# andewx/dieselfluid

Measured on AMD Instinct MI355X. Metric: M particle-steps/sec, 16M-particle WCSPH dam-break; % HBM roofline, higher is better.
Workload: dtype f32; 1 GPU; WCSPH dam-break, 16003008 particles (n3=252), h=2dx, uniform-grid neighbours, density + pressure/viscosity force + integrate + walls, math=fast; particles=16003008, parallelism=single GPU

## Files before the change

### dieselfluid_amd/csrc/kernels_skin.hpp

```cpp
#pragma once

#include "kernels_tiled.hpp"

namespace dsl {

constexpr int kLEntries = 8;
constexpr int kLMaxChunks = 12;
constexpr int kLMaxEntries = kLMaxChunks * kLEntries - 1;
constexpr int kLBlock = 512;
constexpr unsigned int kLGlobal = 0xffffu;
constexpr float kSkinTauSteps = 16.0f;
constexpr int kLQuads = 14;
static_assert(kTRows * kLQuads <= kLBlock, "one quad per lane");

__global__ void k_skin_decide(SkinState* st) {
  const float d = __builtin_sqrtf(__uint_as_float(st->disp2_bits)) * (1.0f + 1.0e-6f);
  const bool rb = st->force != 0 || !(d <= st->budget);
  st->rebuild = rb ? 1 : 0;
  if (st->unlisted * 64 > st->n_live) st->give_up = 1;
  if (rb) {
    st->ids_sel ^= 1;
    st->n_rebuilds += 1;
    st->unlisted = 0;
    st->fields_own = st->fields_padded = 0u;
// ... 216 lines not shown
          tile_run(m, rr, tt.lx, j, je);
          const int g0 = m.row_gs[rr] - m.row_lds[rr];
          const float xi = p.x[g], yi = p.y[g], zi = p.z[g];
          for (int r0 = j; r0 < je; r0 += 32) {
            unsigned int w = 0u;
            const int top = r0 + 31;
            for (int r = r0; r < min(r0 + 32, je); ++r) {
              const float dx = xi - p.x[g0 + r], dy = yi - p.y[g0 + r], dz = zi - p.z[g0 + r];
              const float tq = __builtin_fmaf(-dist2<true>(dx, dy, dz), c.inv_hh, 1.0f);
              if (tq > wide_thr && r != tt.own) w |= 1u << (top - r);
            }
            enqueue(w, top);
          }
        }
      }
      const int n_own = 1 + total;
      const bool fits = masks && !too_many && n_own <= kLMaxChunks * kLEntries;
      if (masks && !fits) st->list_overflow = 1;
      int fields = fits ? n_own : 0;
      const int own_fields = fields;
      int wmax = 0;
#pragma unroll
      for (int bit = 6; bit >= 0; --bit) {
        const int cand = wmax | (1 << bit);
        if (__builtin_amdgcn_ballot_w64(fields >= cand) != 0ull) wmax = cand;
      }
      if constexpr (!SHARED) fields = fits ? wmax : 0;
      atomicAdd(&tile_fields[0], (unsigned int)own_fields);
      atomicAdd(&tile_fields[1], (unsigned int)fields);
      const int nch = (fields + kLEntries - 1) / kLEntries;
      const int nch_wave = (wmax + kLEntries - 1) / kLEntries;
      unsigned int b0 = 0u, b1 = 0u, b2 = 0u, b3 = 0u;
      unsigned int k0 = 0u, k1 = 0u, k2 = 0u, k3 = 0u;
      int qi = 0;
      unsigned int w = 0u, top = 0u;
      unsigned int wn = (fits && nq > 0) ? qword[0][tid] : 0u, tn = (fits && nq > 0) ? qtop[0][tid] : 0u;
      const int nq_live = fits ? nq : 0;
      for (int it = 0; it < nch_wave * kLEntries; ++it) {
        unsigned int entry = pad;
        if (it == 0) {
          entry = 0u;
        } else {
          if (w == 0u && qi < nq_live) {
            w = wn;
            top = tn;
            qi += 1;
            if (qi < nq_live) {
              wn = qword[qi][tid];
              tn = qtop[qi][tid];
            }
          }
          if (w != 0u) {
            const int b = __builtin_ctz(w);
            w &= w - 1u;
            entry = (top - (unsigned int)b) << 4;
          }
        }
        b0 = __builtin_amdgcn_alignbit(b1, b0, 16);
        b1 = __builtin_amdgcn_alignbit(b2, b1, 16);
        b2 = __builtin_amdgcn_alignbit(b3, b2, 16);
        b3 = (b3 >> 16) | (entry << 16);
        if ((it & (kLEntries - 1)) == kLEntries - 1) {
          const int ch = it >> 3;
          if (ch == 0) {
            k0 = b0, k1 = b1, k2 = b2, k3 = b3;
          } else if (ch < nch) {
            lists[(size_t)ch * lstride + g] = make_uint4(b0, b1, b2, b3);
          }
        }
      }
      if (fits) lists[g] = make_uint4((k0 & 0xffff0000u) | (unsigned int)fields, k1, k2, k3);
      else lists[g] = make_uint4(kLGlobal, 0u, 0u, 0u);
    });
    if (have) tile_meta_store(metas[cur ^ 1], table_word);
    sync_lds();
    if (tid == 0) {
      atomicAdd(&st->fields_own, tile_fields[0]);
      atomicAdd(&st->fields_padded, tile_fields[1]);
      tile_fields[0] = tile_fields[1] = 0u;
    }
  }
}

template <int NF, class Load4, class Store>
__device__ __forceinline__ void stage_tile(const TileMeta& m, Load4&& load4, Store&& store) {
  const int t = threadIdx.x, r = t / kLQuads, k = t - r * kLQuads;
  if (r >= kTRows) return;
  const int len = m.row_len[r], gs = m.row_gs[r], ls = m.row_lds[r];
  for (int q = k; 4 * q < len; q += kLQuads) {
    float4 v[NF];
    load4(gs + 4 * q, v);
#pragma unroll
    for (int i = 0; i < 4; ++i) {
      if (4 * q + i < len) {
        float rec[NF];
#pragma unroll
        for (int a = 0; a < NF; ++a) rec[a] = f4_at(v[a], i);
        store(ls + 4 * q + i, rec, true);
      }
    }
  }
  const int npad = m.row_lds[r + 1] - ls - len;
  if (k < npad) {
    float rec[NF];
#pragma unroll
    for (int a = 0; a < NF; ++a) rec[a] = 0.0f;
    store(ls + len + k, rec, false);
  }
}

__device__ __forceinline__ const float4& lds_at(const float4* base, unsigned int byte_offset) {
  return *reinterpret_cast<const float4*>(reinterpret_cast<const char*>(base) + byte_offset);
}

struct Chunk {
  unsigned int x, y, z, w;
};
__device__ __forceinline__ Chunk load_chunk(const uint4* __restrict__ lists, size_t index) {
  const uint4 v = lists[index];
  return Chunk{v.x, v.y, v.z, v.w};
}
__device__ __forceinline__ Chunk pad_chunk(unsigned int pad) {
  const unsigned int w = pad | (pad << 16);
  return Chunk{w, w, w, w};
}
__device__ __forceinline__ unsigned int take_count(Chunk& e, unsigned int pad) {
  const unsigned int cnt = e.x & 0xffffu;
  e.x = (e.x & 0xffff0000u) | pad;
  return cnt;
}
__device__ __forceinline__ int chunks_of(unsigned int cnt) { return cnt == kLGlobal ? 0 : (int)((cnt + kLEntries) >> 3); }

template <class Body>
__device__ __forceinline__ void walk_shared(const uint4* __restrict__ lists, int lstride, int g, unsigned int pad, int sub,
                                            int k, unsigned int fields, Body&& body) {
  const int nch = fields == kLGlobal ? 0 : (int)((fields + kLEntries - 1) >> 3);
  for (int ch = sub; __builtin_amdgcn_ballot_w64(ch < nch) != 0ull; ch += k) {
    Chunk e = pad_chunk(pad);
    if (ch < nch) e = load_chunk(lists, (size_t)ch * lstride + g);
    if (ch == 0) e.x = (e.x & 0xffff0000u) | pad;
    body(e);
  }
}
__device__ __forceinline__ unsigned int shared_fields(const uint4* __restrict__ lists, int g, int sub) {
  unsigned int f = 0u;
  if (sub == 0) f = lists[g].x & 0xffffu;
  return (unsigned int)__shfl((int)f, (int)((threadIdx.x & (kWave - 1)) - sub), kWave);
}

__global__ __launch_bounds__(kLBlock, 4) void k_density_list(DevConsts c, TileGrid tg, const int* __restrict__ desc_of,
                                                             const int* __restrict__ n_tiles, const int* __restrict__ desc,
                                                             const int* __restrict__ cell_start, const SkinState* st,
                                                             CSoa3 pX, CSoa3 pZ, const uint4* __restrict__ lists,
                                                             int lstride, float* __restrict__ rho,
                                                             float* __restrict__ pterm) {
  __shared__ TileMeta metas[2];
  __shared__ float4 A[kTCap];
  const int tid = threadIdx.x;
  const CSoa3 p = st->rebuild ? pZ : pX;
  TileFeed feed(desc_of, *n_tiles);
  int di = 0;
  bool have = feed.pop(di);
  if (have) tile_meta_store(metas[0], tile_meta_request(desc, di));
  for (int cur = 0; have; cur ^= 1) {
    const TileMeta& m = metas[cur];
    sync_lds();
    have = feed.pop(di);
    int table_word = 0;
    if (have) table_word = tile_meta_request(desc, di);
    const int ntarg = m.tprefix[kTB * kTB];
    const bool staged = m.overflow == 0;
    const unsigned int pad = pad_entry(m);
    Chunk q0 = pad_chunk(pad), q1 = q0;
    const bool first_full = ntarg > kLBlock / 2;
    TileTarget tt0{0, 0, 0, 0};
    const int tperm = (tid & ~(kWave - 1)) + b128_group_slot(tid & (kWave - 1));
    if (first_full && tperm < ntarg) {
      tt0 = tile_target(m, tperm);
      q0 = load_chunk(lists, tt0.g);
      q1 = load_chunk(lists, (size_t)lstride + tt0.g);
    }
    if (staged) stage_tile<3>(m, LoadPos4{p}, StoreTileRecord(A, m, c.inv_hh));
    if (have) tile_meta_store(metas[cur ^ 1], table_word);
    sync_lds();
    for_each_target<true, kLBlock>(ntarg, tid, tperm, [&](auto shared_c, int t, int sub, int k) {
      constexpr bool SHARED = decltype(shared_c)::value;
      TileTarget tt;
      unsigned int fields;
      if constexpr (SHARED) {
        tt = tile_target(m, t);
        fields = shared_fields(lists, tt.g, sub);
      } else {
        if (t == tperm) tt = tt0;
        else {
          tt = tile_target(m, t);
          q0 = load_chunk(lists, tt.g);
          q1 = load_chunk(lists, (size_t)lstride + tt.g);
        }
        fields = take_count(q0, pad);
      }
      const int g = tt.g;
      float acc = 0.0f;
      if (staged && fields != kLGlobal) {
        const float4 me = A[tt.own];
        const float two_hh = 2.0f * c.inv_hh;
        const float sx = two_hh * me.x, sy = two_hh * me.y, sz = two_hh * me.z, a0 = 1.0f + me.w;
        float acc0 = 0.0f, acc1 = 0.0f;
        float4 cq[4];
        auto fetch4 = [&](unsigned int w0, unsigned int w1) {
          cq[0] = lds_at(A, w0 & 0xffffu);
          cq[1] = lds_at(A, w0 >> 16);
          cq[2] = lds_at(A, w1 & 0xffffu);
          cq[3] = lds_at(A, w1 >> 16);
        };
        auto sum4 = [&](const float4 (&r)[4]) {
#pragma unroll
          for (int u = 0; u < 4; ++u) {
            const float q = fma_clamp01(r[u].z, sz, __builtin_fmaf(r[u].y, sy, __builtin_fmaf(r[u].x, sx, r[u].w + a0)));
            if (u & 1) acc1 = __builtin_fmaf(q, q, acc1);
            else acc0 = __builtin_fmaf(q, q, acc0);
          }
        };
        if constexpr (SHARED) {
          walk_shared(lists, lstride, g, pad, sub, k, fields, [&](const Chunk& e) {
            fetch4(e.x, e.y);
            float4 c1[4] = {cq[0], cq[1], cq[2], cq[3]};
            fetch4(e.z, e.w);
            sum4(c1);
            sum4(cq);
          });
        } else {
          const int nf = __builtin_amdgcn_readfirstlane((int)fields), nch = (nf + kLEntries - 1) >> 3;
          const uint4* lp = lists + (size_t)2 * lstride + g;
          Chunk e = q0, e1 = q1;
          fetch4(e.x, e.y);
          for (int ch = 0;;) {
            float4 c1[4] = {cq[0], cq[1], cq[2], cq[3]};
            fetch4(e.z, e.w);
            sum4(c1);
            if (8 * ch + 4 >= nf) break;
            const Chunk en = e1;
            if (ch + 2 < nch) e1 = load_chunk(lp, 0);
            lp += lstride;
            float4 c2[4] = {cq[0], cq[1], cq[2], cq[3]};
            fetch4(en.x, en.y);
            sum4(c2);
            e = en;
            ch += 1;
            if (8 * ch >= nf) break;
          }
        }
        acc = acc0 + acc1;
      } else if (sub == 0) {
        const float xi = p.x[g], yi = p.y[g], zi = p.z[g];
        float a = 0.0f;
        for_each_grid_candidate(c, cell_start, xi, yi, zi, [&](int j) {
          if (j == g) return;
          const float dx = xi - p.x[j], dy = yi - p.y[j], dz = zi - p.z[j];
          const float r2 = dist2<true>(dx, dy, dz);
          if (r2 < c.hh) {
            const float q = __builtin_fmaf(-r2, c.inv_hh, 1.0f);
            a = __builtin_fmaf(q, q, a);
          }
        });
        acc = a;
      }
      if constexpr (SHARED) {
        for (int o = 1; o < k; o <<= 1) acc += __shfl_xor(acc, o, kWave);
        if (sub != 0) return;
      }
      acc *= c.mass * c.A;
      rho[g] = acc;
      const float pr = tait_eos<true>(c, acc, c.eos_d0_grad);
      pterm[g] = acc > 0.0f ? dsl_div<true>(pr, acc * acc) : 0.0f;
    });
  }
}

template <bool WANT_G, bool WANT_V, bool QUEUE>
__global__ __launch_bounds__(kLBlock, 4) void k_force_list(DevConsts c, TileGrid tg, const int* __restrict__ desc_of,
                                                           const int* __restrict__ n_tiles, const int* __restrict__ desc,
                                                           const int* __restrict__ cell_start, SkinState* st, CSoa3 pX,
                                                           CSoa3 vX, CSoa3 pZ, CSoa3 vZ, CSoa3 pR, const float* __restrict__ rho,
                                                           const float* __restrict__ pterm,
                                                           const uint4* __restrict__ lists, int lstride, Soa3 pout,
                                                           Soa3 vout, DevStats* stats, int* __restrict__ walk_ctr) {
  __shared__ TileMeta metas[2];
  __shared__ float4 A[kTCap];
  __shared__ float4 B[kTCap];
  __shared__ int feed_slot[2];
  const int tid = threadIdx.x;
  const bool rb = st->rebuild != 0;
  const CSoa3 pin = rb ? pZ : pX, vin = rb ? vZ : vX;
  unsigned int vbits = 0u, fbits = 0u, dbits = 0u;
  typename TileSource<QUEUE>::type feed = TileSource<QUEUE>::make(desc_of, *n_tiles, walk_ctr, feed_slot);
  int di = 0;
  bool have = feed.pop(di);
  if (have) tile_meta_store(metas[0], tile_meta_request(desc, di));
  for (int cur = 0; have; cur ^= 1) {
    const TileMeta& m = metas[cur];
    sync_lds();
    have = feed.pop(di);
    int table_word = 0;
    if (have) table_word = tile_meta_request(desc, di);
    const int ntarg = m.tprefix[kTB * kTB];
    const bool staged = m.overflow == 0;
    const unsigned int pad = pad_entry(m);
    Chunk q0 = pad_chunk(pad), q1 = q0;
    const bool first_full = ntarg > kLBlock / 2;
    TileTarget tt0{0, 0, 0, 0};
    const int tperm = (tid & ~(kWave - 1)) + b128_group_slot(tid & (kWave - 1));
    if (first_full && tperm < ntarg) {
      tt0 = tile_target(m, tperm);
      q0 = load_chunk(lists, tt0.g);
      q1 = load_chunk(lists, (size_t)lstride + tt0.g);
    }
    if (staged)
      stage_tile<8>(
          m,
          [&](int gg, float4* o) {
            o[0] = load4u(pin.x + gg);
            o[1] = load4u(pin.y + gg);
            o[2] = load4u(pin.z + gg);
            o[3] = WANT_G ? load4u(pterm + gg) : make_float4(0.f, 0.f, 0.f, 0.f);
            if constexpr (WANT_V) {
              o[4] = load4u(vin.x + gg);
              o[5] = load4u(vin.y + gg);
              o[6] = load4u(vin.z + gg);
              o[7] = load4u(rho + gg);
            } else {
              o[4] = o[5] = o[6] = o[7] = make_float4(0.f, 0.f, 0.f, 0.f);
            }
          },
          [&](int slot, const float* o, bool real) {
            float4 a = make_float4(kFar, kFar, kFar, 0.f), b = make_float4(0.f, 0.f, 0.f, 0.f);
            if (real && o[0] == o[0] && o[1] == o[1] && o[2] == o[2]) {
              a = make_float4(o[0], o[1], o[2], o[3]);
              if constexpr (WANT_V) b = make_float4(o[4], o[5], o[6], o[7] > 0.0f ? __builtin_amdgcn_rcpf(o[7]) : 0.0f);
            }
            A[slot] = a;
            if constexpr (WANT_V) B[slot] = b;
          });
    if (have) tile_meta_store(metas[cur ^ 1], table_word);
    sync_lds();
    for_each_target<true, kLBlock>(ntarg, tid, tperm, [&](auto shared_c, int t, int sub, int k) {
      constexpr bool SHARED = decltype(shared_c)::value;
      TileTarget tt;
      unsigned int fields;
      if constexpr (SHARED) {
        tt = tile_target(m, t);
        fields = shared_fields(lists, tt.g, sub);
      } else {
        if (t == tperm) tt = tt0;
        else {
          tt = tile_target(m, t);
          q0 = load_chunk(lists, tt.g);
          q1 = load_chunk(lists, (size_t)lstride + tt.g);
        }
        fields = take_count(q0, pad);
      }
      const int g = tt.g;
      float px, py, pz, vx, vy, vz;
      float gx = 0.f, gy = 0.f, gz = 0.f, lx_ = 0.f, ly_ = 0.f, lz_ = 0.f, lw_ = 0.f;
      const bool listed = staged && fields != kLGlobal;
      if (listed) {
        const float4 a = A[tt.own];
        px = a.x, py = a.y, pz = a.z;
        const float pti = WANT_G ? a.w : 0.f;
        if (px == kFar) px = py = pz = __uint_as_float(0x7fc00000u);
        if constexpr (WANT_V) {
          const float4 b = B[tt.own];
          vx = b.x, vy = b.y, vz = b.z;
        } else {
          vx = vin.x[g], vy = vin.y[g], vz = vin.z[g];
        }
        if constexpr (WANT_G || WANT_V) {
          const float ninvh = -c.inv_h;
          auto accum = [&](const float4& ra, const float4& rb2) {
            const float dx = ra.x - px, dyy = ra.y - py, dzz = ra.z - pz;
            float r2 = __builtin_fmaf(dzz, dzz, __builtin_fmaf(dyy, dyy, dx * dx));
            r2 = fmaxf(r2, 1.0e-30f);
            const float rinv = __builtin_amdgcn_rsqf(r2);
            const float dist = r2 * rinv;
            const float q = fma1_clamp01_uniform(dist, ninvh);
            if constexpr (WANT_G) {
              const float kk = (q * q) * (pti + ra.w) * rinv;
              gx = __builtin_fmaf(dx, kk, gx);
              gy = __builtin_fmaf(dyy, kk, gy);
              gz = __builtin_fmaf(dzz, kk, gz);
            }
            if constexpr (WANT_V) {
              const float w = q * rb2.w;
              lx_ = __builtin_fmaf(rb2.x, w, lx_);
              ly_ = __builtin_fmaf(rb2.y, w, ly_);
              lz_ = __builtin_fmaf(rb2.z, w, lz_);
              lw_ += w;
            }
          };
          struct Pair1 {
            float4 a, b;
          };
// ... 123 lines not shown
```

### dieselfluid_amd/csrc/kernels_tiled.hpp

```cpp
#pragma once

#include "kernels_sph.hpp"

namespace dsl {

constexpr int kTH = kTB + 2;
constexpr int kTRows = kTH * kTH;
constexpr int kTBlock = 512;
constexpr int kTPad = 4;
constexpr int kTCap = 2304;
constexpr float kFar = 1.0e15f;
constexpr int kTileLists = 5;
constexpr int kMaskWords = 19;
constexpr int kMaskValid = 9, kMaskHigh = 10;

struct TileMeta {
  int4 trow[kTB * kTB];
  int row_gs[kTRows];
  int row_len[kTRows];
  int row_lds[kTRows + 1];
  int run[kTRows * kTB];
  int tprefix[kTB * kTB + 1];
  int overflow;
  int tile;
  int centre[3];
  int pad_;
  int pprefix[kTB * kTB + 1];
  int pad2_[3];
};
constexpr int kMetaInts = 360;
static_assert(sizeof(TileMeta) == kMetaInts * sizeof(int), "TileMeta is copied as kMetaInts dwords");

__device__ __forceinline__ void sync_lds() {
  asm volatile("s_waitcnt lgkmcnt(0)" ::: "memory");
  __syncthreads();
}

__device__ __forceinline__ int tile_of_list_thread(const TileGrid& tg, int t) {
  if (tg.bx == 0) return t < tg.ntiles ? t : -1;
  const int per = tg.bx * tg.by * tg.bz;
  const int box = t / per, w = t - box * per;
  const int ox = box % tg.nbx, oy = (box / tg.nbx) % tg.nby, oz = box / (tg.nbx * tg.nby);
  const int tx = ox * tg.bx + w % tg.bx, ty = oy * tg.by + (w / tg.bx) % tg.by, tz = oz * tg.bz + w / (tg.bx * tg.by);
  return (tx < tg.tnx && ty < tg.tny && tz < tg.tnz) ? tx + tg.tnx * (ty + tg.tny * tz) : -1;
}

#ifdef DSL_DIAG_STAMPS
__device__ unsigned long long g_diag[32];
#define DSL_STAMP_IF(on, var) const unsigned long long var = (on) ? clock64() : 0ull
#define DSL_STAMP_ADD_IF(on, slot, a, b) \
  if ((on) && threadIdx.x == 0) atomicAdd(&g_diag[slot], (unsigned long long)((b) - (a)))
#else
#define DSL_STAMP_IF(on, var)
#define DSL_STAMP_ADD_IF(on, slot, a, b)
#endif
#define DSL_STAMP(var) DSL_STAMP_IF(true, var)
#define DSL_STAMP_ADD(slot, a, b) DSL_STAMP_ADD_IF(true, slot, a, b)

__global__ __launch_bounds__(kBlock) void k_tile_list(DevConsts c, TileGrid tg, const int* __restrict__ cell_start,
                                                      int* __restrict__ tiles, int* __restrict__ n_tiles,
                                                      int* __restrict__ short_pass_tiles, int* __restrict__ n_live,
                                                      int* __restrict__ desc_of, unsigned int* __restrict__ unordered,
                                                      int unordered_words, int* __restrict__ overfull,
                                                      SkinGate gate = SkinGate{nullptr}) {
  if (gate.closed()) return;
  const int lt = blockIdx.x * kBlock + threadIdx.x;
  if (lt == 0) *overfull = 0;
  if (unordered != nullptr) {
    if (2 * lt < unordered_words) unordered[2 * lt] = 0u;
    if (2 * lt + 1 < unordered_words) unordered[2 * lt + 1] = 0u;
  }
  if (lt == 0 && n_live) *n_live = cell_start[c.ncell];
  const int lane = threadIdx.x & (kWave - 1);
  const int t = tile_of_list_thread(tg, lt);
  int cnt = 0;
  bool in_band = false, in_inner = false, owning = false, ghosts = false;
  if (t >= 0) {
    const int tx = t % tg.tnx, ty = (t / tg.tnx) % tg.tny, tz = t / (tg.tnx * tg.tny);
    const int nx = c.dims[0], ny = c.dims[1], nz = c.dims[2];
    const int xa = tx * kTB, xb = min(xa + kTB, nx);
#pragma unroll
    for (int dz = 0; dz < kTB; ++dz)
#pragma unroll
      for (int dy = 0; dy < kTB; ++dy) {
        const int z = tz * tg.tbz + dz, y = ty * kTB + dy;
        if (dz < tg.tbz && z < nz && y < ny) {
          const int row = (z * ny + y) * nx;
          cnt += cell_start[row + xb] - cell_start[row + xa];
        }
      }
    if (cnt > 0 && c.slab_axis >= 0) {
      const int a = c.slab_axis, ta = a == 0 ? tx : (a == 1 ? ty : tz);
      const int a0 = ta * kTB, a1 = min(a0 + kTB, c.dims[a]);
      owning = max(a0, c.own_c0) < min(a1, c.own_c1);
      ghosts = !owning;
      in_band = owning && (a0 < c.split_cl || a1 > c.split_ch);
      in_inner = owning && max(a0, c.split_cl) < min(a1, c.split_ch);
    }
  }
  __shared__ int wave_count[kBlock / kWave][kTileLists + 1];
  __shared__ int block_base[kTileLists + 1];
  const int wid = threadIdx.x >> 6;
  auto member = [&](int l) {
    return l == 0 ? cnt > 0
                  : (l == 1 ? in_band
                            : (l == 2 ? in_inner
                                      : (l == 3 ? ghosts : (l == 4 ? owning : (cnt > kTBlock || (cnt > 0 && cnt <= kTBlock / 2))))));
  };
  unsigned long long mask_of[kTileLists + 1];
#pragma unroll
  for (int l = 0; l <= kTileLists; ++l) {
    mask_of[l] = __ballot(member(l));
    if (lane == 0) wave_count[wid][l] = __builtin_popcountll(mask_of[l]);
  }
// ... 16 lines not shown
    tiles[(size_t)l * tg.ntiles + pos] = t;
    desc_of[(size_t)l * tg.ntiles + pos] = pos0;
  }
}

struct TileSetupRegs {
  int s[kTH + 1];
};
__device__ __forceinline__ void tile_setup_load(const DevConsts& c, const TileGrid& tg, int tile,
                                                const int* __restrict__ cell_start, TileSetupRegs& r) {
  const int tid = threadIdx.x;
#pragma unroll
  for (int k = 0; k <= kTH; ++k) r.s[k] = 0;
  if (tid >= kTRows) return;
  const int tx = tile % tg.tnx, ty = (tile / tg.tnx) % tg.tny, tz = tile / (tg.tnx * tg.tny);
  const int nx = c.dims[0], ny = c.dims[1], nz = c.dims[2];
  const int ry = tid % kTH, rz = tid / kTH;
  const int y = ty * kTB - 1 + ry, z = tz * tg.tbz - 1 + rz;
  if (y >= 0 && y < ny && z >= 0 && z < nz && rz <= tg.tbz + 1) {
    const int row = (z * ny + y) * nx;
#pragma unroll
    for (int k = 0; k <= kTH; ++k) {
      int x = tx * kTB - 1 + k;
      x = x < 0 ? 0 : (x > nx ? nx : x);
      r.s[k] = cell_start[row + x];
    }
  }
}
constexpr int kQueryRow = 32;
__device__ __forceinline__ void tile_setup_load_counts(const DevConsts& c, const TileGrid& tg, int tile,
                                                       int* __restrict__ qcount, TileSetupRegs& r, bool keep) {
  const int tid = threadIdx.x;
#pragma unroll
  for (int k = 0; k <= kTH; ++k) r.s[k] = 0;
  if (tid >= kTRows) return;
  const int tx = tile % tg.tnx, ty = (tile / tg.tnx) % tg.tny, tz = tile / (tg.tnx * tg.tny);
  const int nx = c.dims[0], ny = c.dims[1], nz = c.dims[2];
  const int ry = tid % kTH, rz = tid / kTH;
  const int y = ty * kTB - 1 + ry, z = tz * kTB - 1 + rz;
  if (ry >= 1 && ry <= kTB && rz >= 1 && rz <= kTB && y < ny && z < nz) {
    const int row = (z * ny + y) * nx;
    int cnt[kTB];
#pragma unroll
    for (int k = 0; k < kTB; ++k) {
      const int x = tx * kTB + k;
      cnt[k] = x < nx ? qcount[row + x] : 0;
    }
#pragma unroll
    for (int k = 0; k < kTB; ++k) {
      const int x = tx * kTB + k;
      if (cnt[k] != 0 && !keep) qcount[row + x] = 0;
      r.s[k + 2] = r.s[k + 1] + min(cnt[k], kQueryRow);
    }
    r.s[kTH] = r.s[kTB + 1];
  }
}

__global__ __launch_bounds__(kWave) void k_tile_desc(DevConsts c, TileGrid tg, const int* __restrict__ cell_start,
                                                     const int* __restrict__ target_start,
                                                     const int* __restrict__ tiles, const int* __restrict__ n_tiles,
                                                     int* __restrict__ desc, int* __restrict__ query_counts = nullptr,
                                                     int lds_cap = kTCap, SkinGate gate = SkinGate{nullptr},
                                                     bool keep_counts = false) {
  if (gate.closed()) return;
  const int n = *n_tiles;
  const int lane = threadIdx.x;
  const int ry = lane % kTH, rz = lane / kTH;
  const bool row = lane < kTRows;
  const bool interior = row && ry >= 1 && ry <= kTB && rz >= 1 && rz <= tg.tbz;
  const bool queries = target_start != cell_start;
  auto table = [&](int item, int tile, const TileSetupRegs& r, const TileSetupRegs& q) {
    TileMeta* out = reinterpret_cast<TileMeta*>(desc + (size_t)item * kMetaInts);
    const int len = r.s[kTH] - r.s[0];
    const int v = row ? len + kTPad : 0;
    const int inc = wave_inclusive_scan(v);
    const int tv = interior ? q.s[kTB + 1] - q.s[1] : 0;
    const int tinc = wave_inclusive_scan(tv);
    int pv = 0;
    if (interior) {
#pragma unroll
      for (int k = 1; k <= kTB; ++k) pv += (q.s[k + 1] - q.s[k] + 1) >> 1;
    }
    const int pinc = wave_inclusive_scan(pv);
    if (row) {
      out->row_gs[lane] = r.s[0];
      out->row_len[lane] = len;
      const int lds0 = inc - v;
      out->row_lds[lane] = lds0;
#pragma unroll
      for (int lx = 1; lx <= kTB; ++lx)
        out->run[lane * kTB + lx - 1] = (lds0 + (r.s[lx - 1] - r.s[0])) | ((lds0 + (r.s[lx + 2] - r.s[0])) << 16);
      if (ry >= 1 && ry <= kTB && rz >= 1 && rz <= kTB) {
        const int ir = (rz - 1) * kTB + (ry - 1), t0 = tinc - tv;
        out->tprefix[ir] = t0;
        out->pprefix[ir] = pinc - pv;
        int first = q.s[1] - t0;
        if (query_counts != nullptr)
          first = (((tile / (tg.tnx * tg.tny)) * kTB + rz - 1) * c.dims[1] + ((tile / tg.tnx) % tg.tny) * kTB + ry - 1) * c.dims[0] +
                  (tile % tg.tnx) * kTB;
        out->trow[ir] = make_int4(first, lds0 + (r.s[1] - r.s[0]) - t0,
                                  (t0 + (q.s[2] - q.s[1])) | ((t0 + (q.s[3] - q.s[1])) << 16), t0 + (q.s[4] - q.s[1]));
      }
      if (lane == kTRows - 1) {
        out->row_lds[kTRows] = inc;
        out->overflow = (inc > lds_cap || tinc > 0xffff) ? 1 : 0;
        out->tprefix[kTB * kTB] = tinc;
        out->pprefix[kTB * kTB] = pinc;
        out->tile = tile;
        out->centre[0] = __float_as_int(c.gmin[0] + ((tile % tg.tnx) * kTB + 0.5f * kTB) * c.cell);
        out->centre[1] = __float_as_int(c.gmin[1] + (((tile / tg.tnx) % tg.tny) * kTB + 0.5f * kTB) * c.cell);
        out->centre[2] = __float_as_int(c.gmin[2] + ((tile / (tg.tnx * tg.tny)) * tg.tbz + 0.5f * tg.tbz) * c.cell);
      }
    }
  };
  for (int item = blockIdx.x; item < n; item += 2 * gridDim.x) {
    const int item2 = item + gridDim.x;
    const bool two = item2 < n;
    const int tile = tiles[item], tile2 = two ? tiles[item2] : 0;
    TileSetupRegs r, r2;
    tile_setup_load(c, tg, tile, cell_start, r);
    if (two) tile_setup_load(c, tg, tile2, cell_start, r2);
    if (query_counts != nullptr) {
      TileSetupRegs q, q2;
      tile_setup_load_counts(c, tg, tile, query_counts, q, keep_counts);
      if (two) tile_setup_load_counts(c, tg, tile2, query_counts, q2, keep_counts);
      table(item, tile, r, q);
      if (two) table(item2, tile2, r2, q2);
    } else if (queries) {
      TileSetupRegs q, q2;
      tile_setup_load(c, tg, tile, target_start, q);
      if (two) tile_setup_load(c, tg, tile2, target_start, q2);
      table(item, tile, r, q);
      if (two) table(item2, tile2, r2, q2);
    } else {
      table(item, tile, r, r);
      if (two) table(item2, tile2, r2, r2);
    }
  }
}

template <bool ROWS>
__global__ __launch_bounds__(kBlock) void k_qtile_list(DevConsts c, TileGrid tg, const int* __restrict__ qstart,
                                                       int* __restrict__ qtiles, int* __restrict__ n_qtiles,
                                                       const DevStats* stats) {
  if (stats->pci_done) return;
  const int lt = blockIdx.x * kBlock + threadIdx.x;
  const int lane = threadIdx.x & (kWave - 1), wid = threadIdx.x >> 6;
  const int t = tile_of_list_thread(tg, lt);
  int cnt = 0;
  if (t >= 0) {
    const int tx = t % tg.tnx, ty = (t / tg.tnx) % tg.tny, tz = t / (tg.tnx * tg.tny);
    const int nx = c.dims[0], ny = c.dims[1], nz = c.dims[2];
    const int xa = tx * kTB, xb = min(xa + kTB, nx);
#pragma unroll
    for (int dz = 0; dz < kTB; ++dz)
#pragma unroll
      for (int dy = 0; dy < kTB; ++dy) {
        const int z = tz * kTB + dz, y = ty * kTB + dy;
        if (z < nz && y < ny) {
          const int row = (z * ny + y) * nx;
          if constexpr (ROWS) {
#pragma unroll
            for (int k = 0; k < kTB; ++k) cnt += xa + k < nx ? qstart[row + xa + k] : 0;
          } else {
            cnt += qstart[row + xb] - qstart[row + xa];
          }
        }
      }
  }
  __shared__ int wave_count[kBlock / kWave];
  __shared__ int block_base;
  const unsigned long long mine = __ballot(cnt > 0);
  if (lane == 0) wave_count[wid] = __builtin_popcountll(mine);
  sync_lds();
  if (threadIdx.x == 0) {
    int total = 0;
    for (int w = 0; w < kBlock / kWave; ++w) total += wave_count[w];
    block_base = total > 0 ? atomicAdd(n_qtiles, total) : 0;
  }
  sync_lds();
  if (cnt > 0) {
    int base = block_base;
    for (int w = 0; w < wid; ++w) base += wave_count[w];
    qtiles[base + __builtin_popcountll(mine & ((1ull << lane) - 1ull))] = t;
  }
}

__device__ __forceinline__ int tile_meta_request(const int* __restrict__ desc, int desc_index) {
  const int tid = threadIdx.x;
  return tid < kMetaInts ? desc[(size_t)desc_index * kMetaInts + tid] : 0;
// ... 161 lines not shown

__device__ __forceinline__ void mask_push(unsigned int& mask, float q) {
  asm("v_cmp_lt_f32_e32 vcc, 0, %1\n\tv_addc_co_u32_e32 %0, vcc, %0, %0, vcc" : "+v"(mask) : "v"(q) : "vcc");
}

__device__ __forceinline__ void mask_push_lt(unsigned int& mask, float a, float b) {
  asm("v_cmp_lt_f32_e32 vcc, %1, %2\n\tv_addc_co_u32_e32 %0, vcc, %0, %0, vcc" : "+v"(mask) : "v"(a), "v"(b) : "vcc");
}

constexpr int kQuadsPerRow = 14;
static_assert(kTRows * kQuadsPerRow <= kTBlock, "one quad per lane");
typedef float f4u __attribute__((ext_vector_type(4), aligned(4)));
__device__ __forceinline__ float4 load4u(const float* __restrict__ p) {
  const f4u v = *reinterpret_cast<const f4u*>(p);
  return make_float4(v.x, v.y, v.z, v.w);
}
__device__ __forceinline__ float f4_at(const float4& v, int i) { return i == 0 ? v.x : (i == 1 ? v.y : (i == 2 ? v.z : v.w)); }

template <int NF>
struct StageRegs {
  float4 v[NF];
};
template <int NF, class Load4>
__device__ __forceinline__ void stage_issue(const TileMeta& m, Load4&& load4, StageRegs<NF>& sr, int vt = -1) {
  const int t = vt < 0 ? (int)threadIdx.x : vt, r = t / kQuadsPerRow, k = t - r * kQuadsPerRow;
  if (r < kTRows && 4 * k < m.row_len[r]) load4(m.row_gs[r] + 4 * k, sr.v);
}
template <int NF, class Load1, class Store>
__device__ __forceinline__ void stage_commit(const TileMeta& m, const StageRegs<NF>& sr, Load1&& load1, Store&& store, int vt = -1) {
  const int t = vt < 0 ? (int)threadIdx.x : vt, r = t / kQuadsPerRow, k = t - r * kQuadsPerRow;
  if (r >= kTRows) return;
  const int len = m.row_len[r], ls = m.row_lds[r];
#pragma unroll
  for (int i = 0; i < 4; ++i) {
    if (4 * k + i < len) {
      float rec[NF];
#pragma unroll
      for (int a = 0; a < NF; ++a) rec[a] = f4_at(sr.v[a], i);
      store(ls + 4 * k + i, rec, true);
    }
  }
  for (int i = 4 * kQuadsPerRow + k; i < len; i += kQuadsPerRow) {
    float rec[NF];
    load1(m.row_gs[r] + i, rec);
    store(ls + i, rec, true);
  }
  const int npad = m.row_lds[r + 1] - ls - len;
  if (k < npad) {
    float rec[NF];
#pragma unroll
    for (int a = 0; a < NF; ++a) rec[a] = 0.0f;
    store(ls + len + k, rec, false);
  }
}
template <int NF, int NC>
__device__ __forceinline__ bool stage_values_ok(const TileMeta& m, const StageRegs<NF>& sr) {
  const int t = threadIdx.x, r = t / kQuadsPerRow, k = t - r * kQuadsPerRow;
  if (r >= kTRows) return true;
  const int len = m.row_len[r];
  bool ok = len <= 4 * kQuadsPerRow;
#pragma unroll
  for (int i = 0; i < 4; ++i) {
    if (4 * k + i < len) {
#pragma unroll
      for (int a = 0; a < NC; ++a) ok = ok && exact_div_ok(f4_at(sr.v[a], i));
    }
  }
  return ok;
}
template <int NF, bool CHECK = false, class Load4, class Load1, class Store>
__device__ __forceinline__ bool stage_rows(const TileMeta& m, Load4&& load4, Load1&& load1, Store&& store) {
  StageRegs<NF> sr;
  DSL_STAMP(s0);
  stage_issue<NF>(m, load4, sr);
  DSL_STAMP(s1);
  DSL_STAMP_ADD(NF == 8 ? 8 : 12, s0, s1);
  stage_commit<NF>(m, sr, load1, store);
  DSL_STAMP(s2);
  DSL_STAMP_ADD(NF == 8 ? 9 : 13, s1, s2);
  if constexpr (CHECK) return stage_values_ok<NF, 3>(m, sr);
  return true;
}

__device__ __forceinline__ bool share_wanted(const int* __restrict__ stats) {
  return (long long)stats[5] * 12 > (long long)stats[0];
}

__device__ __forceinline__ float nine_lane_sum(float v) {
  const int g0 = ((threadIdx.x & (kWave - 1)) / 9) * 9;
  float s = __shfl(v, g0, kWave);
#pragma unroll
  for (int j = 1; j < 9; ++j) s += __shfl(v, g0 + j, kWave);
  return s;
}
template <bool SHARE, int BLOCK = kTBlock, bool NINE = false, class Body>
__device__ __forceinline__ void for_each_target(int ntarg, int tid, int tperm, Body&& body) {
  int tbase = 0;
  for (; SHARE ? ntarg - tbase > BLOCK / 2 : tbase < ntarg; tbase += BLOCK) {
    const int t = tbase + tperm;
    if (t < ntarg) body(std::false_type{}, t, 0, 1);
  }
  if constexpr (SHARE)
  while (tbase < ntarg) {
    const int rem = ntarg - tbase;
    if constexpr (NINE) {
      constexpr int kGroups = (BLOCK / kWave) * 7;
      if (rem > BLOCK / 16 && rem <= 2 * kGroups) {
        const int lane = tid & (kWave - 1);
        const int t = (tid / kWave) * 7 + lane / 9;
        if (lane < 63 && t < rem) body(std::true_type{}, tbase + t, lane % 9, 9);
        tbase += min(rem, kGroups);
        continue;
      }
    }
    const int shift = rem > BLOCK / 4 ? 1 : (rem > BLOCK / 8 ? 2 : (rem > BLOCK / 16 ? 3 : 4));
    const int t = tid >> shift;
    if (t < rem) body(std::true_type{}, tbase + t, tid & ((1 << shift) - 1), 1 << shift);
    tbase += min(rem, BLOCK >> shift);
  }
}

struct LoadPos4 {
  CSoa3 p;
  __device__ __forceinline__ void operator()(int g, float4* o) const {
    o[0] = load4u(p.x + g);
    o[1] = load4u(p.y + g);
    o[2] = load4u(p.z + g);
  }
};
struct LoadPos1 {
  CSoa3 p;
  __device__ __forceinline__ void operator()(int g, float* o) const {
    o[0] = p.x[g];
    o[1] = p.y[g];
    o[2] = p.z[g];
  }
};

__device__ __forceinline__ float4 tile_record(const float* o, bool real, float ox, float oy, float oz, float inv_hh) {
  float4 v = make_float4(0.0f, 0.0f, 0.0f, -1.0e30f);
  if (real) {
    const float x = o[0] - ox, y = o[1] - oy, z = o[2] - oz;
    v = make_float4(x, y, z, -inv_hh * __builtin_fmaf(z, z, __builtin_fmaf(y, y, x * x)));
  }
  return v;
}
struct StoreTileRecord {
  float4* img;
  float ox, oy, oz, inv_hh;
  __device__ __forceinline__ StoreTileRecord(float4* image, const TileMeta& m, float inv_hh_)
      : img(image), ox(__int_as_float(m.centre[0])), oy(__int_as_float(m.centre[1])), oz(__int_as_float(m.centre[2])), inv_hh(inv_hh_) {}
  __device__ __forceinline__ void operator()(int slot, const float* o, bool real) const { img[slot] = tile_record(o, real, ox, oy, oz, inv_hh); }
};

template <bool SHARED, class F>
__device__ __forceinline__ void for_each_run(int srow, int sub, int k, F&& f) {
  if constexpr (!SHARED) {
    int ri = 0;
#pragma unroll 1
    for (int dz = -kTH; dz <= kTH; dz += kTH) {
#pragma unroll 1
      for (int dy = -1; dy <= 1; ++dy, ++ri) f(ri, srow + dz + dy);
    }
  } else {
#pragma unroll 1
    for (int ri = sub; ri < 9; ri += k) f(ri, srow + (ri / 3 - 1) * kTH + (ri % 3 - 1));
// ... 43 lines not shown
  for_each_run<false>(qrow, 0, 1, [&](int, int rr) {
    int j, je;
    tile_run(m, rr, lx, j, je);
    for (; j + 4 < je; j += 8) {
      test4(j);
      test4(j + 4);
    }
    if (j < je) test4(j);
  });
  return acc + acc1;
}
__device__ __forceinline__ float densityf_global(const DevConsts& c, const int* cell_start, const CSoa3& p, float qx,
                                                 float qy, float qz) {
  float density = c.W0;
  for_each_grid_candidate(c, cell_start, qx, qy, qz, [&](int j) {
    const float dx = qx - p.x[j], dy = qy - p.y[j], dz = qz - p.z[j];
    const float r2 = dist2<true>(dx, dy, dz);
    if (r2 < c.hh) {
      const float q = __builtin_fmaf(-r2, c.inv_hh, 1.0f);
      density = __builtin_fmaf(c.mass * c.A, q * q, density);
    }
  });
  return density;
}
__device__ __forceinline__ void pci_accumulate(const DevConsts& c, float* press, int g, float density, unsigned int& ebits) {
  const float density_error = density - c.ref_density;
  const float abs_err = density_error * __builtin_amdgcn_rcpf(c.ref_density);
  press[g] += density_error * c.delta;
  const unsigned int eb = nonneg_bits(abs_err);
  ebits = eb > ebits ? eb : ebits;
}

template <bool STAMPS, class Commit, class Sweep>
__device__ __forceinline__ void sweep_tiles_double_buffered(TileFeed& feed, const int* desc, TileMeta* metas,
                                                            float4 (*Abuf)[kTCap], const LoadPos4& load4, Commit&& commit,
                                                            Sweep&& sweep) {
  int di = 0;
  bool have = feed.pop(di);
  if (!have) return;
  tile_meta_store(metas[0], tile_meta_request(desc, di));
  bool have_next = feed.pop(di);
  int table_word = have_next ? tile_meta_request(desc, di) : 0;
  sync_lds();
  {
    StageRegs<3> sr;
    if (!metas[0].overflow) {
      stage_issue<3>(metas[0], load4, sr);
      commit(metas[0], sr, Abuf[0]);
    }
  }
  if (have_next) tile_meta_store(metas[1], table_word);
  int mc = 0, mn = 1, mnn = 2;
  for (int cur = 0; have; cur ^= 1) {
    DSL_STAMP_IF(STAMPS, d0);
    sync_lds();
    DSL_STAMP_IF(STAMPS, d1);
    DSL_STAMP_ADD_IF(STAMPS, 4, d0, d1);
    StageRegs<3> sr;
    bool have_nn = false, stage_next = false;
    table_word = 0;
    if (have_next) {
      stage_next = metas[mn].overflow == 0;
      if (stage_next) stage_issue<3>(metas[mn], load4, sr);
      have_nn = feed.pop(di);
      if (have_nn) table_word = tile_meta_request(desc, di);
    }
    DSL_STAMP_IF(STAMPS, d1b);
    DSL_STAMP_ADD_IF(STAMPS, 12, d1, d1b);
    sweep(metas[mc], Abuf[cur]);
    DSL_STAMP_IF(STAMPS, d4);
    if (stage_next) commit(metas[mn], sr, Abuf[cur ^ 1]);
    if (have_nn) tile_meta_store(metas[mnn], table_word);
    DSL_STAMP_IF(STAMPS, d5);
    DSL_STAMP_ADD_IF(STAMPS, 13, d4, d5);
    have = have_next;
    have_next = have_nn;
    const int t = mc;
    mc = mn;
    mn = mnn;
    mnn = t;
  }
}

template <int BLOCK, class Body>
__device__ __forceinline__ void sweep_tiles_pair(const DevConsts& c, TileFeed& feed, const int* desc, TileMeta* metas,
                                                 float4* A, const CSoa3& p, Body&& body) {
  const int tid = threadIdx.x;
  const LoadPos4 load4{p};
  const LoadPos1 load1{p};
  auto meta_request = [&](int desc_index, int (&w)[2]) {
#pragma unroll
    for (int k = 0; k < 2; ++k) {
      const int i = tid + k * BLOCK;
      w[k] = i < kMetaInts ? desc[(size_t)desc_index * kMetaInts + i] : 0;
    }
  };
  auto meta_store = [&](TileMeta& m, const int (&w)[2]) {
#pragma unroll
    for (int k = 0; k < 2; ++k) {
      const int i = tid + k * BLOCK;
      if (i < kMetaInts) reinterpret_cast<int*>(&m)[i] = w[k];
    }
  };
  int di = 0;
  bool have = feed.pop(di);
  if (!have) return;
  {
    int w[2];
    meta_request(di, w);
    meta_store(metas[0], w);
  }
  for (int cur = 0; have; cur ^= 1) {
    TileMeta& m = metas[cur];
    sync_lds();
    have = feed.pop(di);
    int tw[2] = {0, 0};
    if (have) meta_request(di, tw);
    const bool ovf = m.overflow != 0;
    if (!ovf) {
      const StoreTileRecord store(A, m, c.inv_hh);
      StageRegs<3> sr0, sr1;
      stage_issue<3>(m, load4, sr0, tid);
      stage_issue<3>(m, load4, sr1, tid + BLOCK);
      stage_commit<3>(m, sr0, load1, store, tid);
      stage_commit<3>(m, sr1, load1, store, tid + BLOCK);
    }
    if (have) meta_store(metas[cur ^ 1], tw);
    sync_lds();
    body(m, ovf);
  }
}
struct MaskQueue {
  unsigned int mm, n1, n2;
  int top, tp1, tp2;
  __device__ __forceinline__ void shift() {
    mm = n1;
    top = tp1;
    n1 = n2;
    tp1 = tp2;
    n2 = 0u;
  }
  __device__ __forceinline__ int take(int own, int pad_rec, bool& counts) {
    const bool has = mm != 0u;
    const int b = 31 - __builtin_clz(mm | 1u);
    const int idx = has ? top - b : pad_rec;
    mm = has ? (mm & ~(1u << b)) : 0u;
    counts = has && idx != own;
    if (mm == 0u) shift();
    return idx;
  }
};

template <bool SHARE, bool EXACT = false>
__global__ __launch_bounds__(kTBlock, 4) void k_density_tiled(DevConsts c, TileGrid tg, const int* __restrict__ desc_of,
                                                          const int* __restrict__ n_tiles, const int* __restrict__ desc,
                                                          const int* __restrict__ cell_start, Bnd bnd, CSoa3 p,
                                                          float* __restrict__ rho, float* __restrict__ pterm,
                                                          unsigned int* __restrict__ nmask, int mstride) {
#ifdef DSL_DENSITY_SINGLE_BUFFER
  constexpr bool DB = false;
#else
  constexpr bool DB = !EXACT;
#endif
  __shared__ TileMeta metas[DB ? 3 : 2];
  __shared__ float4 Abuf[DB ? 2 : 1][kTCap];
  __shared__ float4 R[EXACT ? kTCap : 1];
  const int tid = threadIdx.x, lane = tid & (kWave - 1);
  static_assert(!(EXACT && SHARE), "the exact sum is sequential: one lane per target");
  if (!EXACT && c.slab_axis < 0 && share_wanted(n_tiles) != SHARE) return;
  const LoadPos4 load4{p};
  const LoadPos1 load1{p};
  auto commit = [&](const TileMeta& mt, const StageRegs<3>& sr, float4* img) {
    const float ox = __int_as_float(mt.centre[0]), oy = __int_as_float(mt.centre[1]), oz = __int_as_float(mt.centre[2]);
    stage_commit<3>(mt, sr, load1, [&](int slot, const float* o, bool real) {
      const float4 v = tile_record(o, real, ox, oy, oz, c.inv_hh);
      if constexpr (EXACT) {
        img[slot] = real ? make_float4(o[0], o[1], o[2], 0.0f) : make_float4(kFar, kFar, kFar, 0.0f);
        R[slot] = v;
      } else {
        img[slot] = v;
      }
    });
  };
  auto sweep = [&](const TileMeta& m, const float4* __restrict__ A, bool force_global) {
    DSL_STAMP(d2);
    const bool ovf = m.overflow != 0 || force_global;
    const int ntarg = m.tprefix[kTB * kTB];
    const int tperm = (tid & ~(kWave - 1)) + b128_group_slot(lane);
    for_each_target<SHARE>(ntarg, tid, tperm, [&](auto shared_c, int t, int sub, int k) {
      constexpr bool SHARED = decltype(shared_c)::value;
      const TileTarget tt = tile_target(m, t);
      const int srow = tt.srow, g = tt.g, lx = tt.lx;
      float acc = 0.0f, acc1 = 0.0f, self_term = 1.0f;
      if constexpr (EXACT) {
        if (!ovf) {
          const int own = tt.own;
          const float4 me = A[own];
          const int pad_rec = m.row_lds[1] - kTPad;
          float density = 0.0f;
          const float4 mer = R[own];
          const float two_hh = 2.0f * c.inv_hh;
          const float qsx = two_hh * mer.x, qsy = two_hh * mer.y, qsz = two_hh * mer.z, qa0 = 1.0f + mer.w;
          const float reach = 4.0f * c.h;
          const bool far_lane = !(fabsf(mer.x) <= reach && fabsf(mer.y) <= reach && fabsf(mer.z) <= reach);
          const bool prefilter = __builtin_amdgcn_ballot_w64(far_lane) == 0ull;
          const ExactDivisor Dhh = exact_divisor_uniform(c.hh);
          auto add = [&](const float4& cnd, bool counts) {
            const float dx = me.x - cnd.x, dy = me.y - cnd.y, dz = me.z - cnd.z;
// ... 178 lines not shown
  TileFeed feed(desc_of, *n_tiles);
  if constexpr (DB) {
    sweep_tiles_double_buffered<true>(feed, desc, metas, Abuf, load4, commit,
                                      [&](const TileMeta& m, const float4* __restrict__ A) { sweep(m, A, false); });
  } else {
    int di = 0;
    bool have = feed.pop(di);
    if (!have) return;
    tile_meta_store(metas[0], tile_meta_request(desc, di));
    for (int cur = 0; have; cur ^= 1) {
      TileMeta& m = metas[cur];
      sync_lds();
      have = feed.pop(di);
      int table_word = 0;
      if (have) table_word = tile_meta_request(desc, di);
      bool unsafe = EXACT && !exact_div_ok(c.h);
      if (!m.overflow) {
        StageRegs<3> sr;
        stage_issue<3>(m, load4, sr);
        commit(m, sr, Abuf[0]);
        if constexpr (EXACT) unsafe |= !stage_values_ok<3, 3>(m, sr);
      }
      if (have) tile_meta_store(metas[cur ^ 1], table_word);
      bool force_global = false;
      if constexpr (EXACT) {
        asm volatile("s_waitcnt lgkmcnt(0)" ::: "memory");
        force_global = __syncthreads_or(unsafe ? 1 : 0) != 0;
      }
      else sync_lds();
      sweep(m, Abuf[0], force_global);
    }
  }
}

constexpr int kPBlock = 256;
#ifndef DSL_PAIR_NINE
#define DSL_PAIR_NINE 1
#endif
constexpr bool kPairNine = DSL_PAIR_NINE != 0;
struct PairSlot {
  int srow, lx, g, own;
  int rowbase, j;
  bool two;
};
__device__ __forceinline__ PairSlot pair_slot(const TileMeta& m, int u) {
  const int ir = tile_row_of(m.pprefix, u);
  const int4 w = m.trow[ir];
  const int b1 = m.tprefix[ir], b2 = w.z & 0xffff, b3 = (int)((unsigned)w.z >> 16), b4 = w.w, b5 = m.tprefix[ir + 1];
  const int n1 = (b2 - b1 + 1) >> 1, n2 = (b3 - b2 + 1) >> 1, n3 = (b4 - b3 + 1) >> 1;
  int q = u - m.pprefix[ir];
  int lx = 1, begin = b1, end = b2;
  if (q >= n1) {
    q -= n1, lx = 2, begin = b2, end = b3;
    if (q >= n2) {
      q -= n2, lx = 3, begin = b3, end = b4;
      if (q >= n3) q -= n3, lx = 4, begin = b4, end = b5;
    }
  }
  const int t0 = begin + 2 * q;
  PairSlot r;
  r.srow = (ir / kTB + 1) * kTH + (ir % kTB + 1);
  r.lx = lx;
  r.g = w.x + t0;
  r.own = w.y + t0;
  r.rowbase = w.x;
  r.j = 2 * q;
  r.two = t0 + 1 < end;
  return r;
}

template <bool SHARE, bool WIDE = false>
__global__ __launch_bounds__(kPBlock, 4) void k_density_pair(DevConsts c, TileGrid tg, const int* __restrict__ desc_of,
                                                             const int* __restrict__ n_tiles, const int* __restrict__ desc,
                                                             const int* __restrict__ cell_start, Bnd bnd, CSoa3 p,
                                                             float* __restrict__ rho, float* __restrict__ pterm,
                                                             unsigned int* __restrict__ nmask, int mstride,
                                                             float wide_thr = 0.0f, SkinGate gate = SkinGate{nullptr}) {
  __shared__ TileMeta metas[2];
  __shared__ float4 A[kTCap];
  const int tid = threadIdx.x;
  if (gate.closed()) return;
  if (!WIDE && c.slab_axis < 0 && share_wanted(n_tiles) != SHARE) return;
  TileFeed feed(desc_of, *n_tiles);
  sweep_tiles_pair<kPBlock>(c, feed, desc, metas, A, p, [&](const TileMeta& m, bool ovf) {
    if (ovf) {
      if constexpr (!WIDE) {
        const int ntarg = m.tprefix[kTB * kTB];
        for (int t = tid; t < ntarg; t += kPBlock) {
          const int g = tile_target(m, t).g;
          const float a = bnd.is(g) ? 0.0f : density_global_fast(c, cell_start, p, g);
          store_density_fast(c, bnd, rho, pterm, g, a);
        }
      }
      return;
    }
    const int nslots = m.pprefix[kTB * kTB];
    for_each_target<SHARE, kPBlock, kPairNine>(nslots, tid, tid, [&](auto shared_c, int u, int sub, int k) {
      constexpr bool SHARED = decltype(shared_c)::value;
      const PairSlot ps = pair_slot(m, u);
      const int srow = ps.srow, lx = ps.lx, g0 = ps.g;
      const bool two = ps.two;
      float acc[2] = {0.0f, 0.0f}, accb[2] = {0.0f, 0.0f}, self_term[2] = {1.0f, 1.0f};
      const float4 me0 = A[ps.own];
      float4 me1 = A[ps.own + (two ? 1 : 0)];
      self_term[0] = (me0.x == me0.x && me0.y == me0.y && me0.z == me0.z) ? 1.0f : 0.0f;
      self_term[1] = (me1.x == me1.x && me1.y == me1.y && me1.z == me1.z) ? 1.0f : 0.0f;
      const float two_hh = 2.0f * c.inv_hh;
      const float sx0 = two_hh * me0.x, sy0 = two_hh * me0.y, sz0 = two_hh * me0.z, a00 = 1.0f + me0.w;
      const float sx1 = two_hh * me1.x, sy1 = two_hh * me1.y, sz1 = two_hh * me1.z;
      const float a01 = two ? 1.0f + me1.w : -1.0e30f;
      auto sweep_run = [&](int ri, int rr) {
        int j, je;
        tile_run(m, rr, lx, j, je);
        unsigned int mask0 = 0u, mask1 = 0u;
        auto test4 = [&](int jj) {
#pragma unroll
          for (int v = 0; v < 4; ++v) {
            const float4 cnd = A[jj + v];
            if constexpr (WIDE) {
              const float t0 = __builtin_fmaf(cnd.z, sz0, __builtin_fmaf(cnd.y, sy0, __builtin_fmaf(cnd.x, sx0, cnd.w + a00)));
              const float t1 = __builtin_fmaf(cnd.z, sz1, __builtin_fmaf(cnd.y, sy1, __builtin_fmaf(cnd.x, sx1, cnd.w + a01)));
              mask_push_lt(mask0, wide_thr, t0);
              mask_push_lt(mask1, wide_thr, t1);
              continue;
            }
            const float q0 = fma_clamp01(cnd.z, sz0, __builtin_fmaf(cnd.y, sy0, __builtin_fmaf(cnd.x, sx0, cnd.w + a00)));
            const float q1 = fma_clamp01(cnd.z, sz1, __builtin_fmaf(cnd.y, sy1, __builtin_fmaf(cnd.x, sx1, cnd.w + a01)));
            mask_push(mask0, q0);
            mask_push(mask1, q1);
            if (v & 1) {
              accb[0] = __builtin_fmaf(q0, q0, accb[0]);
              accb[1] = __builtin_fmaf(q1, q1, accb[1]);
            } else {
              acc[0] = __builtin_fmaf(q0, q0, acc[0]);
              acc[1] = __builtin_fmaf(q1, q1, acc[1]);
            }
          }
        };
        auto sweep_to = [&](int jend) {
          for (; j + 4 < jend; j += 8) {
            test4(j);
            test4(j + 4);
          }
          if (j < jend) {
            test4(j);
            j += 4;
          }
        };
        const int j32 = j + 32;
        sweep_to(min(je, j32));
        nmask[(size_t)ri * mstride + g0] = mask0;
        if (two) nmask[(size_t)ri * mstride + g0 + 1] = mask1;
        if (je > j32) {
          mask0 = mask1 = 0u;
          sweep_to(je);
          nmask[(size_t)(kMaskHigh + ri) * mstride + g0] = mask0;
          if (two) nmask[(size_t)(kMaskHigh + ri) * mstride + g0 + 1] = mask1;
        }
      };
      for_each_run<SHARED>(srow, sub, k, sweep_run);
      acc[0] += accb[0];
      acc[1] += accb[1];
      if constexpr (WIDE) return;
      if constexpr (SHARED) {
        if (k == 9) {
          acc[0] = nine_lane_sum(acc[0]);
          acc[1] = nine_lane_sum(acc[1]);
// ... 932 lines not shown
```

Measured before the change: 8216 M particle-steps/s.

## Deal tile staging quads across all lanes via per-row quad prefix

Adds a per-row quad prefix (qprefix) to the tile metadata, built during tile setup. Tile staging then assigns each lane a global quad index across the whole tile instead of a fixed row/lane mapping, so work is balanced across the block regardless of row lengths. Padding stores are split into a separate pass. This grows TileMeta from 360 to 376 dwords, adds a small per-lane row search, and affects the skin, force and wide density paths.

```diff
diff --git a/dieselfluid_amd/csrc/kernels_skin.hpp b/dieselfluid_amd/csrc/kernels_skin.hpp
--- a/dieselfluid_amd/csrc/kernels_skin.hpp
+++ b/dieselfluid_amd/csrc/kernels_skin.hpp
@@ -322,8 +322,20 @@
   }
 }
 
-template <int NF, class Load4, class Store>
+template <int NF, bool DEALT, class Load4, class Store>
 __device__ __forceinline__ void stage_tile(const TileMeta& m, Load4&& load4, Store&& store) {
+  if constexpr (DEALT) {
+    const int nq = __builtin_amdgcn_readfirstlane((int)m.qprefix[kTRows]);
+    auto pass = [&](int base) {
+      StageRegs<NF> sr;
+      const StageWhere w = stage_issue_dealt<NF>(m, load4, sr, base + (int)threadIdx.x, nq);
+      stage_commit_dealt<NF>(sr, w, store);
+    };
+    pass(0);
+    for (int base = kLBlock; base < nq; base += kLBlock) pass(base);
+    stage_pads<NF>(m, store, threadIdx.x);
+    return;
+  }
   const int t = threadIdx.x, r = t / kLQuads, k = t - r * kLQuads;
   if (r >= kTRows) return;
   const int len = m.row_len[r], gs = m.row_gs[r], ls = m.row_lds[r];
@@ -420,7 +432,7 @@
       q0 = load_chunk(lists, tt0.g);
       q1 = load_chunk(lists, (size_t)lstride + tt0.g);
     }
-    if (staged) stage_tile<3>(m, LoadPos4{p}, StoreTileRecord(A, m, c.inv_hh));
+    if (staged) stage_tile<3, (kStageDealt & 1) != 0>(m, LoadPos4{p}, StoreTileRecord(A, m, c.inv_hh));
     if (have) tile_meta_store(metas[cur ^ 1], table_word);
     sync_lds();
     for_each_target<true, kLBlock>(ntarg, tid, tperm, [&](auto shared_c, int t, int sub, int k) {
@@ -556,7 +568,7 @@
       q1 = load_chunk(lists, (size_t)lstride + tt0.g);
     }
     if (staged)
-      stage_tile<8>(
+      stage_tile<8, (kStageDealt & 2) != 0>(
           m,
           [&](int gg, float4* o) {
             o[0] = load4u(pin.x + gg);
diff --git a/dieselfluid_amd/csrc/kernels_tiled.hpp b/dieselfluid_amd/csrc/kernels_tiled.hpp
--- a/dieselfluid_amd/csrc/kernels_tiled.hpp
+++ b/dieselfluid_amd/csrc/kernels_tiled.hpp
@@ -26,10 +26,11 @@
   int centre[3];
   int pad_;
   int pprefix[kTB * kTB + 1];
-  int pad2_[3];
+  unsigned short qprefix[kTRows + 2];
 };
-constexpr int kMetaInts = 360;
+constexpr int kMetaInts = 376;
 static_assert(sizeof(TileMeta) == kMetaInts * sizeof(int), "TileMeta is copied as kMetaInts dwords");
+static_assert(kMetaInts % 4 == 0 && kMetaInts <= kTBlock, "one dword per lane of a 512-thread block, two of a 256-thread one");
 
 __device__ __forceinline__ void sync_lds() {
   asm volatile("s_waitcnt lgkmcnt(0)" ::: "memory");
@@ -212,9 +213,12 @@
       for (int k = 1; k <= kTB; ++k) pv += (q.s[k + 1] - q.s[k] + 1) >> 1;
     }
     const int pinc = wave_inclusive_scan(pv);
+    const int qv = row ? (len + 3) >> 2 : 0;
+    const int qinc = wave_inclusive_scan(qv);
     if (row) {
       out->row_gs[lane] = r.s[0];
       out->row_len[lane] = len;
+      out->qprefix[lane] = (unsigned short)(qinc - qv);
       const int lds0 = inc - v;
       out->row_lds[lane] = lds0;
 #pragma unroll
@@ -236,6 +240,8 @@
         out->overflow = (inc > lds_cap || tinc > 0xffff) ? 1 : 0;
         out->tprefix[kTB * kTB] = tinc;
         out->pprefix[kTB * kTB] = pinc;
+        out->qprefix[kTRows] = (unsigned short)qinc;
+        out->qprefix[kTRows + 1] = 0;
         out->tile = tile;
         out->centre[0] = __float_as_int(c.gmin[0] + ((tile % tg.tnx) * kTB + 0.5f * kTB) * c.cell);
         out->centre[1] = __float_as_int(c.gmin[1] + (((tile / tg.tnx) % tg.tny) * kTB + 0.5f * kTB) * c.cell);
@@ -563,6 +569,54 @@
   return true;
 }
 
+#ifndef DSL_STAGE_DEALT
+#define DSL_STAGE_DEALT 7
+#endif
+constexpr int kStageDealt = DSL_STAGE_DEALT;
+__device__ __forceinline__ int tile_quad_row(const TileMeta& m, int t) {
+  int r0 = 0;
+#pragma unroll
+  for (int i = 1; i < 6; ++i) r0 += (t >= (int)m.qprefix[6 * i]) ? 6 : 0;
+  int r = r0;
+#pragma unroll
+  for (int i = 1; i < 6; ++i) r += (t >= (int)m.qprefix[r0 + i]) ? 1 : 0;
+  return r;
+}
+struct StageWhere {
+  int slot, n;
+};
+template <int NF, class Load4>
+__device__ __forceinline__ StageWhere stage_issue_dealt(const TileMeta& m, Load4&& load4, StageRegs<NF>& sr, int t, int nq) {
+  if (t >= nq) return StageWhere{0, 0};
+  const int r = tile_quad_row(m, t), k = t - (int)m.qprefix[r];
+  load4(m.row_gs[r] + 4 * k, sr.v);
+  return StageWhere{m.row_lds[r] + 4 * k, m.row_len[r] - 4 * k};
+}
+template <int NF, class Store>
+__device__ __forceinline__ void stage_commit_dealt(const StageRegs<NF>& sr, const StageWhere& w, Store&& store) {
+#pragma unroll
+  for (int i = 0; i < 4; ++i) {
+    if (i < w.n) {
+      float rec[NF];
+#pragma unroll
+      for (int a = 0; a < NF; ++a) rec[a] = f4_at(sr.v[a], i);
+      store(w.slot + i, rec, true);
+    }
+  }
+}
+template <int NF, class Store>
+__device__ __forceinline__ void stage_pads(const TileMeta& m, Store&& store, int vt) {
+  const int r = vt / kQuadsPerRow, k = vt - r * kQuadsPerRow;
+  if (r >= kTRows) return;
+  const int end = m.row_lds[r] + m.row_len[r];
+  if (k < m.row_lds[r + 1] - end) {
+    float rec[NF];
+#pragma unroll
+    for (int a = 0; a < NF; ++a) rec[a] = 0.0f;
+    store(end + k, rec, false);
+  }
+}
+
 __device__ __forceinline__ bool share_wanted(const int* __restrict__ stats) {
   return (long long)stats[5] * 12 > (long long)stats[0];
 }
@@ -772,7 +826,7 @@
   }
 }
 
-template <int BLOCK, class Body>
+template <int BLOCK, bool DEALT = false, class Body>
 __device__ __forceinline__ void sweep_tiles_pair(const DevConsts& c, TileFeed& feed, const int* desc, TileMeta* metas,
                                                  float4* A, const CSoa3& p, Body&& body) {
   const int tid = threadIdx.x;
@@ -809,11 +863,26 @@
     const bool ovf = m.overflow != 0;
     if (!ovf) {
       const StoreTileRecord store(A, m, c.inv_hh);
-      StageRegs<3> sr0, sr1;
-      stage_issue<3>(m, load4, sr0, tid);
-      stage_issue<3>(m, load4, sr1, tid + BLOCK);
-      stage_commit<3>(m, sr0, load1, store, tid);
-      stage_commit<3>(m, sr1, load1, store, tid + BLOCK);
+      if constexpr (DEALT) {
+        const int nq = __builtin_amdgcn_readfirstlane((int)m.qprefix[kTRows]);
+        auto pass = [&](int base) {
+          StageRegs<3> sr0, sr1;
+          const StageWhere w0 = stage_issue_dealt<3>(m, load4, sr0, base + tid, nq);
+          const StageWhere w1 = stage_issue_dealt<3>(m, load4, sr1, base + tid + BLOCK, nq);
+          stage_commit_dealt<3>(sr0, w0, store);
+          stage_commit_dealt<3>(sr1, w1, store);
+        };
+        pass(0);
+        for (int base = 2 * BLOCK; base < nq; base += 2 * BLOCK) pass(base);
+        stage_pads<3>(m, store, tid);
+        stage_pads<3>(m, store, tid + BLOCK);
+      } else {
+        StageRegs<3> sr0, sr1;
+        stage_issue<3>(m, load4, sr0, tid);
+        stage_issue<3>(m, load4, sr1, tid + BLOCK);
+        stage_commit<3>(m, sr0, load1, store, tid);
+        stage_commit<3>(m, sr1, load1, store, tid + BLOCK);
+      }
     }
     if (have) meta_store(metas[cur ^ 1], tw);
     sync_lds();
@@ -1158,7 +1227,7 @@
   if (gate.closed()) return;
   if (!WIDE && c.slab_axis < 0 && share_wanted(n_tiles) != SHARE) return;
   TileFeed feed(desc_of, *n_tiles);
-  sweep_tiles_pair<kPBlock>(c, feed, desc, metas, A, p, [&](const TileMeta& m, bool ovf) {
+  sweep_tiles_pair<kPBlock, WIDE && (kStageDealt & 4) != 0>(c, feed, desc, metas, A, p, [&](const TileMeta& m, bool ovf) {
     if (ovf) {
       if constexpr (!WIDE) {
         const int ntarg = m.tprefix[kTB * kTB];
```

After: 8346 M particle-steps/s, median of 6. 1.02x the previous value.
